# Pixie8888/R3DFSSeg

Hardware: NVIDIA B200
Metric: MPTI episodes/s (2-way 5-shot, 2048 pts) (higher is better)
Workload: dtype f32

## Files before the change

r3dfsseg_b200/csrc/lp.cu:

```cuda
#include <cooperative_groups.h>

#include <stdlib.h>

#include "common.cuh"
#include "lp.cuh"

namespace cg = cooperative_groups;

#define GD_BM 128
#define GD_BN 64
#define GD_BK 16

template <int ROWS, int KC>
__device__ __forceinline__ void lp_load_tile_T(float* __restrict__ dst,
                                               const float* __restrict__ src, int ld, int64_t row0,
                                               int64_t rows_end, int k0, int k_end) {
  constexpr int KG = KC / 8;
  constexpr int PAIRS = (ROWS / 4) * KG;
  const int lane = threadIdx.x & 31, w = threadIdx.x >> 5;
  const int nw = blockDim.x >> 5;
  const int r_lo = lane & 3, k_lo = lane >> 2;
  for (int p = w; p < PAIRS; p += nw) {
    int kg = p % KG, rg = p / KG;
    int row = 4 * rg + r_lo, kk = 8 * kg + k_lo;
// ... 911 lines not shown
  float v[NCV];
#pragma unroll
  for (int c = 0; c < NCV; ++c) v[c] = warp_sum(part[c]);
  if (lane == 0) {
#pragma unroll
    for (int c = 0; c < NCV; ++c) s_warp[w * CG_MAXC + c] = v[c];
  }
  __syncthreads();
  const int par = xcnt & 1;
  if (tid < NCV) {
    float s = 0.f;
    for (int q = 0; q < n_warps; ++q) s += s_warp[q * CG_MAXC + tid];
    for (int r = 0; r < CL; ++r) {
      float* dst = cluster.map_shared_rank(&ex->slot[par][rank][tid], r);
      *dst = s;
    }
  }
  cluster.sync();
#pragma unroll
  for (int c = 0; c < NCV; ++c) {
    float s = 0.f;
    for (int r = 0; r < CL; ++r) s += ex->slot[par][r][c];
    total[c] = s;
  }
  ++xcnt;
}

__global__ __launch_bounds__(256) void cg_hist_kernel(const int32_t* __restrict__ rowptr,
                                                      const int32_t* __restrict__ rowlen,
                                                      const uint8_t* __restrict__ valid,
                                                      const uint16_t* __restrict__ mcol, int nn,
                                                      int k, int32_t* __restrict__ rowmax) {
  const int g = blockIdx.y;
  const int i = blockIdx.x * 8 + (threadIdx.x >> 5);
  if (i >= nn) return;
  const int lane = threadIdx.x & 31;
  const int64_t vb = (int64_t)g * nn;
  int mx = 0;
  if (valid[vb + i]) {
    const int L = rowlen[vb + i];
    const uint16_t* c = mcol + vb * lp_rowcap(k) + rowptr[vb + i];
    int cnt[8] = {0, 0, 0, 0, 0, 0, 0, 0};
    for (int t0 = 0; t0 < L; t0 += 32) {
      const int t = t0 + lane;
      const int res = t < L ? (int)(c[t] & 7) : -1;
#pragma unroll
      for (int b = 0; b < 8; ++b) cnt[b] += __popc(__ballot_sync(0xffffffffu, res == b));
    }
#pragma unroll
    for (int b = 0; b < 8; ++b) mx = max(mx, cnt[b]);
  }
  if (lane == 0) rowmax[vb + i] = mx;
}

__global__ __launch_bounds__(1024) void cg_pack_kernel(
    const int32_t* __restrict__ rowptr, const int32_t* __restrict__ rowlen,
    const int32_t* __restrict__ rowmax, const uint16_t* __restrict__ mcol,
    const float* __restrict__ mval, int nn, int k, int64_t pk_cap, int32_t* __restrict__ tab_all,
    int32_t* __restrict__ flags, uint2* __restrict__ pcol, float4* __restrict__ pval) {
  extern __shared__ __align__(16) unsigned char pk_smem[];
  uint32_t* s_key = reinterpret_cast<uint32_t*>(pk_smem);
  int* s_pre = reinterpret_cast<int*>(s_key + 4096);
  int* s_prx = s_pre + 8192;
  __shared__ int s_scan[2][32];
  __shared__ int s_tot[2];
  __shared__ int s_rng[2];
  __shared__ int s_wtot[32], s_wbase[32];
  const int CL = gridDim.x, rank = blockIdx.x, g = blockIdx.y;
  const int tid = threadIdx.x, lane = tid & 31, w = tid >> 5;
  const int64_t vb = (int64_t)g * nn;
  const int32_t* rp = rowptr + vb;
  const int32_t* rl = rowlen + vb;
  const int32_t* rmx = rowmax + vb;
  const uint16_t* mc = mcol + vb * lp_rowcap(k);
  const float* mv = mval + vb * lp_rowcap(k);
  int32_t* tab = tab_all + (size_t)(g * CL + rank) * CG_TAB_INTS;
  for (int e = tid; e < CG_TAB_HDR + 32 * CG_MAXPASS * 2; e += 1024) tab[e] = 0;
  {
    int nseg[8], run = 0, runx = 0;
#pragma unroll
    for (int u = 0; u < 8; ++u) {
      const int i = tid * 8 + u;
      nseg[u] = i < nn ? (rmx[i] + CG_SEGR - 1) / CG_SEGR : 0;
      run += nseg[u];
      runx += nseg[u] > 1 ? nseg[u] : 0;
    }
    int inc = run, incx = runx;
#pragma unroll
    for (int o = 1; o < 32; o <<= 1) {
      const int a = __shfl_up_sync(0xffffffffu, inc, o), ax = __shfl_up_sync(0xffffffffu, incx, o);
      if (lane >= o) {
        inc += a;
        incx += ax;
      }
    }
    if (lane == 31) {
      s_scan[0][w] = inc;
      s_scan[1][w] = incx;
    }
    __syncthreads();
    if (w == 0) {
      int v = s_scan[0][lane], vx = s_scan[1][lane];
      int i2 = v, ix2 = vx;
#pragma unroll
      for (int o = 1; o < 32; o <<= 1) {
        const int a = __shfl_up_sync(0xffffffffu, i2, o), ax = __shfl_up_sync(0xffffffffu, ix2, o);
        if (lane >= o) {
          i2 += a;
          ix2 += ax;
        }
      }
      s_scan[0][lane] = i2 - v;
      s_scan[1][lane] = ix2 - vx;
      if (lane == 31) {
        s_tot[0] = i2;
        s_tot[1] = ix2;
      }
    }
    if (tid == 0) {
      s_rng[0] = nn;
      s_rng[1] = 0;
    }
    __syncthreads();
    int pre = s_scan[0][w] + inc - run, prex = s_scan[1][w] + incx - runx;
#pragma unroll
    for (int u = 0; u < 8; ++u) {
      const int i = tid * 8 + u;
      if (i < nn) {
        s_pre[i] = pre;
        s_prx[i] = prex;
      }
      pre += nseg[u];
      prex += nseg[u] > 1 ? nseg[u] : 0;
    }
  }
  __syncthreads();
  const int NV = s_tot[0];
  for (int i = tid; i < nn; i += 1024) {
    const int owner = NV > 0 ? min(CL - 1, (int)((int64_t)s_pre[i] * CL / NV)) : (i * CL) / nn;
    if (owner == rank) {
      atomicMin(&s_rng[0], i);
      atomicMax(&s_rng[1], i + 1);
    }
  }
  __syncthreads();
  const int lo = min(s_rng[0], s_rng[1]), hi = s_rng[1];
  const int pre_lo = lo < nn ? s_pre[lo] : NV, prx_lo = lo < nn ? s_prx[lo] : s_tot[1];
  const int nv = (hi < nn ? s_pre[hi] : NV) - pre_lo;
  const int nx = (hi < nn ? s_prx[hi] : s_tot[1]) - prx_lo;
  const int passes = (nv + CGC_MAXT - 1) / CGC_MAXT;
  const int64_t share = pk_cap / CL;
  bool bad = passes > CG_MAXPASS || nx > CG_MAXPART || hi - lo > 8191;
  int npow = 32;
  while (npow < nv) npow <<= 1;
  if (!bad) {
    for (int i = tid; i < npow; i += 1024) s_key[i] = 0;
    __syncthreads();
    for (int i = lo + tid; i < hi; i += 1024) {
      const int mx = rmx[i];
      const int ns = (mx + CG_SEGR - 1) / CG_SEGR;
      if (ns > 255) bad = true;
      for (int sg = 0; sg < ns && sg < 256; ++sg) {
        const int ranks = min(CG_SEGR, mx - sg * CG_SEGR);
        s_key[s_pre[i] - pre_lo + sg] =
            ((uint32_t)(2 * ranks) << 21) | ((uint32_t)(i - lo) << 8) | (uint32_t)sg;
      }
    }
  }
  bad = __syncthreads_or(bad);
  if (!bad) {
    for (int ksz = 2; ksz <= npow; ksz <<= 1)
      for (int j = ksz >> 1; j > 0; j >>= 1) {
        for (int i = tid; i < npow; i += 1024) {
          const int ixj = i ^ j;
          if (ixj > i) {
            const uint32_t x = s_key[i], y = s_key[ixj];
            const bool desc = (i & ksz) == 0;
            if (desc ? x < y : x > y) {
              s_key[i] = y;
              s_key[ixj] = x;
            }
          }
        }
        __syncthreads();
      }
    if (tid < 32) {
      int tot = 0;
      for (int p = 0; p < passes; ++p) {
        const int i0 = p * CGC_MAXT + tid * 32;
        tot += i0 < nv ? (int)(s_key[i0] >> 21) * 32 : 0;
      }
      s_wtot[tid] = tot;
    }
    __syncthreads();
    if (tid == 0) {
      int run = 0;
      for (int q = 0; q < 32; ++q) {
        s_wbase[q] = run;
        run += s_wtot[q];
      }
      s_tot[0] = run;
    }
    __syncthreads();
    if (s_tot[0] > share) bad = true;
  }
  if (tid == 0) {
    tab[0] = lo;
    tab[1] = hi;
    tab[2] = bad ? 0 : passes;
    tab[3] = nx;
    if (bad) atomicOr(&flags[g], 1);
  }
  if (bad) return;
  for (int e = tid; e < CG_MAXPASS * CGC_MAXT; e += 1024) {
    const int p = e / CGC_MAXT, t = e % CGC_MAXT;
    const int i = p * CGC_MAXT + t;
    int m0 = -1, m1 = 0;
    if (p < passes && i < nv) {
      const uint32_t key = s_key[i];
      const int rloc = (int)((key >> 8) & 0x1fffu), sg = (int)(key & 0xffu);
      const int ns = (rmx[lo + rloc] + CG_SEGR - 1) / CG_SEGR;
      m0 = (rloc << 8) | sg;
      m1 = (ns << 16) | (ns > 1 ? s_prx[lo + rloc] - prx_lo : 0);
    }
    tab[CG_TAB_HDR + 32 * CG_MAXPASS * 2 + 2 * e + 0] = m0;
    tab[CG_TAB_HDR + 32 * CG_MAXPASS * 2 + 2 * e + 1] = m1;
  }
  uint2* gc = pcol + (int64_t)g * pk_cap + rank * share;
  float4* gv = pval + (int64_t)g * pk_cap + rank * share;
  int base = s_wbase[w];
  for (int p = 0; p < passes; ++p) {
    const int i0 = p * CGC_MAXT + w * 32;
    const int rounds = i0 < nv ? (int)(s_key[i0] >> 21) : 0;
    if (lane == 0) {
      tab[CG_TAB_HDR + (w * CG_MAXPASS + p) * 2 + 0] = (int)(rank * share) + base;
      tab[CG_TAB_HDR + (w * CG_MAXPASS + p) * 2 + 1] = rounds;
    }
    for (int r = 0; r < rounds; ++r) {
      const unsigned t0 = (unsigned)(lane + 4 * r);
      uint2 c2;
      c2.x = (t0 & 7u) | (((t0 + 1) & 7u) << 16);
      c2.y = ((t0 + 2) & 7u) | (((t0 + 3) & 7u) << 16);
      gc[base + r * 32 + lane] = c2;
      gv[base + r * 32 + lane] = make_float4(0.f, 0.f, 0.f, 0.f);
    }
    __syncwarp();
    uint16_t* c16 = reinterpret_cast<uint16_t*>(gc + base);
    float* v32 = reinterpret_cast<float*>(gv + base);
    int my_L = 0, my_ptr = 0, my_sg = 0;
    if (i0 + lane < nv) {
      const uint32_t key = s_key[i0 + lane];
      const int row = lo + (int)((key >> 8) & 0x1fffu);
      my_L = rl[row];
      my_ptr = rp[row];
      my_sg = (int)(key & 0xffu);
    }
    const int n_here = min(32, nv - i0);
    for (int l = 0; l < n_here; ++l) {
      const int L = __shfl_sync(0xffffffffu, my_L, l), sg = __shfl_sync(0xffffffffu, my_sg, l);
      const int ptr = __shfl_sync(0xffffffffu, my_ptr, l);
      const int r_lo = sg * CG_SEGR, r_hi = r_lo + CG_SEGR;
      const uint16_t* c = mc + ptr;
      const float* v = mv + ptr;
      int seen[8] = {0, 0, 0, 0, 0, 0, 0, 0};
      int col_n = lane < L ? (int)c[lane] : -1;
      float val_n = lane < L ? v[lane] : 0.f;
      for (int t0 = 0; t0 < L; t0 += 32) {
        const int col = col_n;
        const float val = val_n;
        const int tn = t0 + 32 + lane;
        col_n = tn < L ? (int)c[tn] : -1;
        val_n = tn < L ? v[tn] : 0.f;
        const int res = col >= 0 ? (col & 7) : -1;
        int rho = -1;
#pragma unroll
        for (int b = 0; b < 8; ++b) {
          const uint32_t m = __ballot_sync(0xffffffffu, res == b);
          if (res == b) rho = seen[b] + __popc(m & ((1u << lane) - 1));
          seen[b] += __popc(m);
        }
        if (rho >= r_lo && rho < r_hi) {
          const int step = 8 * (rho - r_lo) + ((res - l) & 7);
          const int64_t d = ((int64_t)(step >> 2) * 32 + l) * 4 + (step & 3);
          c16[d] = (uint16_t)col;
          v32[d] = val;
        }
        int done_all = 1;
#pragma unroll
        for (int b = 0; b < 8; ++b) done_all &= seen[b] >= r_hi;
        if (done_all) break;
      }
    }
    __syncwarp();
    base += rounds * 32;
  }
}

template <int NCV>
__global__ __launch_bounds__(CGC_MAXT, 1) void lp_cg_kernel(
    const int32_t* __restrict__ rowptr, const int32_t* __restrict__ rowlen,
    const uint16_t* __restrict__ mcol, const float* __restrict__ mval,
    const uint8_t* __restrict__ valid, int nn, int k,
    const float* __restrict__ Y, int nc, float alpha, float tol, int max_iter,
    float* __restrict__ Z, float* __restrict__ X, float* __restrict__ R, float* __restrict__ Pv,
    float* __restrict__ AP, int32_t* __restrict__ iters_out, float* __restrict__ resid_out,
    const int32_t* __restrict__ tab_all, const int32_t* __restrict__ flags,
    const uint2* __restrict__ pcol, const float4* __restrict__ pval, int64_t pk_cap) {
  cg::cluster_group cluster = cg::this_cluster();
  const int CL = cluster.num_blocks(), rank = cluster.block_rank();
  const int g = blockIdx.y;
  extern __shared__ __align__(16) float Ps[];
  __shared__ CgExchange ex;
  __shared__ float s_warp[(CGC_MAXT / 32) * CG_MAXC];
  float* s_split = Ps + (size_t)nn * NCV;
  const int tid = threadIdx.x, lane = tid & 31, w = tid >> 5, T = blockDim.x;
  const int64_t vb = (int64_t)g * nn;
  const uint8_t* vg = valid + vb;
  const float* Yg = Y + vb * nc;
  float* Zg = Z + vb * nc;
  float* Xg = X + vb * NCV;
  float* Rg = R + vb * NCV;
  float* Pg = Pv + vb * NCV;
  float* APg = AP + vb * NCV;
  const int32_t* tab = tab_all + (size_t)(g * CL + rank) * CG_TAB_INTS;
  const int lo = tab[0], hi = tab[1];
  const int nloc = hi - lo;
  int xcnt = 0;

  float part[NCV], bb[NCV], rs[NCV], tot[NCV];
#pragma unroll
  for (int c = 0; c < NCV; ++c) part[c] = 0.f;
  for (int jj = tid; jj < nloc; jj += T) {
    const int row = lo + jj;
    const bool ok = vg[row];
#pragma unroll
    for (int c = 0; c < NCV; ++c) {
      const float y = (ok && c < nc) ? Yg[(int64_t)row * nc + c] : 0.f;
      Xg[(int64_t)row * NCV + c] = 0.f;
      Rg[(int64_t)row * NCV + c] = y;
      Pg[(int64_t)row * NCV + c] = y;
      APg[(int64_t)row * NCV + c] = 0.f;
      part[c] = fmaf(y, y, part[c]);
    }
  }
  cg_allreduce<NCV>(cluster, &ex, s_warp, part, xcnt, bb);
  bool done[NCV];
  bool all_done = true;
#pragma unroll
  for (int c = 0; c < NCV; ++c) {
    rs[c] = bb[c];
    done[c] = !(bb[c] > 0.f);
    all_done = all_done && done[c];
  }
  const float tol2 = tol * tol;
  const bool packed = flags[g] == 0;
  const int passes = packed ? tab[2] : 0;
  const bool any_split = packed && tab[3] > 0;
  const int32_t* t_slice = tab + CG_TAB_HDR + w * CG_MAXPASS * 2;
  const int32_t* t_thread = tab + CG_TAB_HDR + 32 * CG_MAXPASS * 2 + 2 * tid;
  const uint2* gc = pcol + (int64_t)g * pk_cap;
  const float4* gv = pval + (int64_t)g * pk_cap;
  int it = 0;
  while (!all_done && it < max_iter) {
    {
      const float4* src = reinterpret_cast<const float4*>(Pg);
      float4* dst = reinterpret_cast<float4*>(Ps);
      const int n4 = nn * (NCV / 4);
      for (int i = tid; i < n4; i += T) dst[i] = __ldcg(src + i);
    }
    __syncthreads();
#pragma unroll
    for (int c = 0; c < NCV; ++c) part[c] = 0.f;
    if (packed) {
      constexpr unsigned SH = NCV == 4 ? 4 : 5;
      const unsigned char* Pb = reinterpret_cast<const unsigned char*>(Ps);
#pragma unroll
      for (int p = 0; p < passes; ++p) {
        const int rounds = __ldg(t_slice + 2 * p + 1);
        if (rounds == 0) continue;
        const int sbase = __ldg(t_slice + 2 * p);
        const uint2* c2 = gc + sbase + lane;
        const float4* v4 = gv + sbase + lane;
        float acc[NCV];
#pragma unroll
        for (int c = 0; c < NCV; ++c) acc[c] = 0.f;
        auto fma4 = [&](float wgt, unsigned byte_off) {
#pragma unroll
          for (int q = 0; q < NCV / 4; ++q) {
            const float4 p4 = *reinterpret_cast<const float4*>(Pb + byte_off + 16 * q);
            acc[4 * q + 0] = fmaf(wgt, p4.x, acc[4 * q + 0]);
            acc[4 * q + 1] = fmaf(wgt, p4.y, acc[4 * q + 1]);
            acc[4 * q + 2] = fmaf(wgt, p4.z, acc[4 * q + 2]);
            acc[4 * q + 3] = fmaf(wgt, p4.w, acc[4 * q + 3]);
          }
        };
        auto consume = [&](const uint2& c, const float4& v) {
          fma4(v.x, (c.x & 0xffffu) << SH);
          fma4(v.y, (c.x >> 16) << SH);
          fma4(v.z, (c.y & 0xffffu) << SH);
          fma4(v.w, (c.y >> 16) << SH);
        };
        uint2 ca = __ldcs(c2), cb = __ldcs(c2 + 32);
        float4 va = __ldcs(v4), vb4 = __ldcs(v4 + 32);
        for (int r = 2; r < rounds; r += 2) {
          const uint2 na = __ldcs(c2 + r * 32), nb = __ldcs(c2 + r * 32 + 32);
          const float4 wa = __ldcs(v4 + r * 32), wb = __ldcs(v4 + r * 32 + 32);
          consume(ca, va);
          consume(cb, vb4);
          ca = na;
          cb = nb;
          va = wa;
          vb4 = wb;
        }
        consume(ca, va);
        consume(cb, vb4);
        const int m0 = __ldg(t_thread + 2 * p * CGC_MAXT), m1 = __ldg(t_thread + 2 * p * CGC_MAXT + 1);
        if (m0 >= 0) {
          if ((m1 >> 16) == 1) {
            const int row = lo + (m0 >> 8);
#pragma unroll
            for (int c = 0; c < NCV; ++c) {
              const float pv = Ps[(size_t)row * NCV + c];
              const float ap = pv - alpha * acc[c];
              APg[(int64_t)row * NCV + c] = ap;
              part[c] = fmaf(pv, ap, part[c]);
            }
          } else {
            float* dst = s_split + (size_t)((m1 & 0xffff) + (m0 & 0xff)) * NCV;
#pragma unroll
            for (int c = 0; c < NCV; ++c) dst[c] = acc[c];
          }
        }
      }
      if (any_split) {
        __syncthreads();
        for (int p = 0; p < passes; ++p) {
          const int m0 = __ldg(t_thread + 2 * p * CGC_MAXT), m1 = __ldg(t_thread + 2 * p * CGC_MAXT + 1);
          if (m0 >= 0 && (m1 >> 16) > 1 && (m0 & 0xff) == 0) {
            const int row = lo + (m0 >> 8), ns = m1 >> 16;
            const float* src = s_split + (size_t)(m1 & 0xffff) * NCV;
#pragma unroll
            for (int c = 0; c < NCV; ++c) {
              float sum = 0.f;
              for (int sg = 0; sg < ns; ++sg) sum += src[sg * NCV + c];
              const float pv = Ps[(size_t)row * NCV + c];
              const float ap = pv - alpha * sum;
              APg[(int64_t)row * NCV + c] = ap;
              part[c] = fmaf(pv, ap, part[c]);
            }
          }
        }
      }
    } else {
      const int32_t* rp = rowptr + vb;
      const int32_t* rl = rowlen + vb;
      const uint16_t* mc = mcol + vb * lp_rowcap(k);
      const float* mv = mval + vb * lp_rowcap(k);
      for (int row = lo + w; row < hi; row += T >> 5) {
        if (!vg[row]) continue;
        float acc[NCV];
#pragma unroll
        for (int c = 0; c < NCV; ++c) acc[c] = 0.f;
        const int L = rl[row];
        const uint16_t* crow = mc + rp[row];
        const float* vrow = mv + rp[row];
        for (int t = lane; t < L; t += 32) {
          const int cj = (int)crow[t];
          const float cv = vrow[t];
#pragma unroll
          for (int c = 0; c < NCV; ++c) acc[c] = fmaf(cv, Ps[(size_t)cj * NCV + c], acc[c]);
        }
#pragma unroll
        for (int c = 0; c < NCV; ++c) {
          const float sum = warp_sum(acc[c]);
          const float pv = Ps[(size_t)row * NCV + c];
          const float ap = pv - alpha * sum;
          if (lane == 0) {
            APg[(int64_t)row * NCV + c] = ap;
            part[c] = fmaf(pv, ap, part[c]);
          }
        }
      }
    }
    cg_allreduce<NCV>(cluster, &ex, s_warp, part, xcnt, tot);
    float a[NCV];
#pragma unroll
    for (int c = 0; c < NCV; ++c) a[c] = (!done[c] && tot[c] > 0.f) ? rs[c] / tot[c] : 0.f;
#pragma unroll
    for (int c = 0; c < NCV; ++c) part[c] = 0.f;
    for (int jj = tid; jj < nloc; jj += T) {
      const int row = lo + jj;
#pragma unroll
      for (int c = 0; c < NCV; ++c) {
        const int64_t o = (int64_t)row * NCV + c;
        const float r = Rg[o] - a[c] * APg[o];
        Xg[o] = fmaf(a[c], Ps[o], Xg[o]);
        Rg[o] = r;
        part[c] = fmaf(r, r, part[c]);
      }
    }
    cg_allreduce<NCV>(cluster, &ex, s_warp, part, xcnt, tot);
    float beta[NCV];
    all_done = true;
#pragma unroll
    for (int c = 0; c < NCV; ++c) {
      beta[c] = (!done[c] && rs[c] > 0.f) ? tot[c] / rs[c] : 0.f;
      if (!done[c]) {
        rs[c] = tot[c];
        if (tot[c] <= tol2 * bb[c]) done[c] = true;
      }
      all_done = all_done && done[c];
    }
    for (int jj = tid; jj < nloc; jj += T) {
      const int row = lo + jj;
#pragma unroll
      for (int c = 0; c < NCV; ++c)
        if (!done[c]) {
          const int64_t o = (int64_t)row * NCV + c;
          Pg[o] = fmaf(beta[c], Ps[o], Rg[o]);
        }
    }
    ++it;
    cluster.sync();
  }
  for (int jj = tid; jj < nloc; jj += T) {
    const int row = lo + jj;
    for (int c = 0; c < nc; ++c) Zg[(int64_t)row * nc + c] = Xg[(int64_t)row * NCV + c];
  }
  if (rank == 0 && tid == 0) {
    if (iters_out) iters_out[g] = it;
    if (resid_out) {
      float m = 0.f;
#pragma unroll
      for (int c = 0; c < NCV; ++c)
        if (bb[c] > 0.f) m = fmaxf(m, sqrtf(rs[c] / bb[c]));
      resid_out[g] = m;
    }
  }
  cluster.sync();
}

template <int NCV>
static int launch_cg(int CL, int G, size_t smem, cudaStream_t st, const int32_t* rowptr,
                     const int32_t* rowlen, const uint16_t* mcol, const float* mval,
                     const uint8_t* valid, int nn, int k, const float* Y, int nc,
                     float alpha, float tol, int max_iter, float* Z, float* X, float* R, float* P,
                     float* AP, int32_t* iters_out, float* resid_out, void* scratch,
                     size_t scratch_bytes) {
  cudaError_t e = cudaFuncSetAttribute(lp_cg_kernel<NCV>,
                                       cudaFuncAttributeMaxDynamicSharedMemorySize, 200 * 1024);
  if (e != cudaSuccess) return (int)e;
  if (CL > 8) {
    e = cudaFuncSetAttribute(lp_cg_kernel<NCV>, cudaFuncAttributeNonPortableClusterSizeAllowed, 1);
    if (e != cudaSuccess) return (int)e;
  }
  const int T = CGC_MAXT;
  smem += sizeof(float) * (size_t)CG_MAXPART * NCV;
  cudaLaunchConfig_t cfg = {};
  cfg.gridDim = dim3(CL, G, 1);
  cfg.blockDim = dim3(T, 1, 1);
  cfg.dynamicSmemBytes = smem;
  cfg.stream = st;
  cudaLaunchAttribute attr[1];
  attr[0].id = cudaLaunchAttributeClusterDimension;
  attr[0].val.clusterDim.x = CL;
  attr[0].val.clusterDim.y = 1;
  attr[0].val.clusterDim.z = 1;
  cfg.attrs = attr;
  cfg.numAttrs = 1;
  {
    int n_clusters = 0;
    e = cudaOccupancyMaxActiveClusters(&n_clusters, lp_cg_kernel<NCV>, &cfg);
    if (e != cudaSuccess || n_clusters < 1) {
      (void)cudaGetLastError();
      return -1000;
    }
  }
  const int64_t pk_cap = lp_pack_groups(nn, k);
  const size_t tab_bytes = align_up(sizeof(int32_t) * (size_t)G * CL * CG_TAB_INTS, 256);
  const size_t flg_bytes = align_up(sizeof(int32_t) * (size_t)G * (1 + nn), 256);
  const size_t col_bytes = align_up(sizeof(uint2) * (size_t)G * pk_cap, 256);
  const size_t val_bytes = align_up(sizeof(float4) * (size_t)G * pk_cap, 256);
  if (!scratch || scratch_bytes < tab_bytes + flg_bytes + col_bytes + val_bytes)
    return R3DFS_E_WORKSPACE;
  unsigned char* sp = reinterpret_cast<unsigned char*>(scratch);
  int32_t* tab = reinterpret_cast<int32_t*>(sp);
  int32_t* flags = reinterpret_cast<int32_t*>(sp + tab_bytes);
  uint2* pcol = reinterpret_cast<uint2*>(sp + tab_bytes + flg_bytes);
  float4* pval = reinterpret_cast<float4*>(sp + tab_bytes + flg_bytes + col_bytes);
  e = cudaMemsetAsync(flags, 0, sizeof(int32_t) * (size_t)G, st);
  if (e != cudaSuccess) return (int)e;
  e = cudaFuncSetAttribute(cg_pack_kernel, cudaFuncAttributeMaxDynamicSharedMemorySize, CG_PK_SMEM);
  if (e != cudaSuccess) return (int)e;
  int32_t* rowmax = flags + G;
  cg_hist_kernel<<<dim3((nn + 7) / 8, G), 256, 0, st>>>(rowptr, rowlen, valid, mcol, nn, k, rowmax);
  R3DFS_CHECK_LAUNCH();
  cg_pack_kernel<<<dim3(CL, G), 1024, CG_PK_SMEM, st>>>(rowptr, rowlen, rowmax, mcol, mval, nn, k,
                                                       pk_cap, tab, flags, pcol, pval);
  R3DFS_CHECK_LAUNCH();
  const int32_t* tabc = tab;
  const int32_t* flc = flags;
  const uint2* pc = pcol;
  const float4* pv = pval;
  e = cudaLaunchKernelEx(&cfg, lp_cg_kernel<NCV>, rowptr, rowlen, mcol, mval, valid, nn, k, Y, nc,
                         alpha, tol, max_iter, Z, X, R, P, AP, iters_out, resid_out, tabc, flc, pc,
                         pv, pk_cap);
  if (e != cudaSuccess) return (int)e;
  ++r3dfs_launches;
  return 0;
}

#define GCG_SLOT 8
#define GCG_MAX_GS 160

__device__ __forceinline__ unsigned ld_acquire_u32(const unsigned* p) {
  unsigned v;
  asm volatile("ld.acquire.gpu.global.u32 %0, [%1];" : "=r"(v) : "l"(p) : "memory");
  return v;
}

__device__ __forceinline__ void group_barrier(unsigned* cnt, unsigned& target, int GS) {
  __syncthreads();
  if (threadIdx.x == 0) {
    target += (unsigned)GS;
    __threadfence();
    atomicAdd(cnt, 1u);
    while (ld_acquire_u32(cnt) < target) {
    }
    __threadfence();
  }
  __syncthreads();
}

template <int NCV>
__device__ __forceinline__ void group_allreduce(float* s_warp, float* s_slot, const float* part,
                                                float* slots, int rank, int GS, unsigned* cnt,
                                                unsigned& target, int& phase, float* total) {
  const int tid = threadIdx.x, lane = tid & 31, w = tid >> 5;
  float v[NCV];
#pragma unroll
  for (int c = 0; c < NCV; ++c) v[c] = warp_sum(part[c]);
  if (lane == 0) {
#pragma unroll
    for (int c = 0; c < NCV; ++c) s_warp[w * CG_MAXC + c] = v[c];
  }
  __syncthreads();
  float* my = slots + ((size_t)(phase & 1) * GS + rank) * GCG_SLOT;
  if (tid < NCV) {
    float s = 0.f;
    for (int q = 0; q < CG_THREADS / 32; ++q) s += s_warp[q * CG_MAXC + tid];
    __stcg(my + tid, s);
  }
  group_barrier(cnt, target, GS);
  const float* all = slots + (size_t)(phase & 1) * GS * GCG_SLOT;
  if (tid < GS) {
#pragma unroll
    for (int q = 0; q < NCV / 4; ++q)
      reinterpret_cast<float4*>(s_slot + tid * GCG_SLOT)[q] =
          __ldcg(reinterpret_cast<const float4*>(all + (size_t)tid * GCG_SLOT) + q);
  }
  __syncthreads();
#pragma unroll
  for (int c = 0; c < NCV; ++c) total[c] = 0.f;
  for (int r = 0; r < GS; ++r) {
#pragma unroll
    for (int q = 0; q < NCV / 4; ++q) {
      const float4 t4 = reinterpret_cast<const float4*>(s_slot + r * GCG_SLOT)[q];
      total[4 * q + 0] += t4.x;
      total[4 * q + 1] += t4.y;
      total[4 * q + 2] += t4.z;
      total[4 * q + 3] += t4.w;
    }
  }
  ++phase;
}

template <int NCV, bool SMEM>
__device__ __forceinline__ void cg_row_product(const uint16_t* crow, const float* vrow, int L,
                                               int lane, const float* Ps, float* acc) {
  int t0 = 0;
  for (; t0 + 256 <= L; t0 += 256) {
    int cj[8];
    float cv[8];
#pragma unroll
    for (int u = 0; u < 8; ++u) {
      const int t = t0 + lane + 32 * u;
      cj[u] = (int)crow[t];
      cv[u] = vrow[t];
    }
#pragma unroll
    for (int u = 0; u < 8; ++u) {
#pragma unroll
      for (int q = 0; q < NCV / 4; ++q) {
        const float4 p4 = *reinterpret_cast<const float4*>(Ps + (int64_t)cj[u] * NCV + 4 * q);
        acc[4 * q + 0] = fmaf(cv[u], p4.x, acc[4 * q + 0]);
        acc[4 * q + 1] = fmaf(cv[u], p4.y, acc[4 * q + 1]);
        acc[4 * q + 2] = fmaf(cv[u], p4.z, acc[4 * q + 2]);
        acc[4 * q + 3] = fmaf(cv[u], p4.w, acc[4 * q + 3]);
      }
    }
  }
  if (t0 < L) {
    const int nU = (L - t0 + 31) >> 5;
    int cj[8];
    float cv[8];
#pragma unroll
    for (int u = 0; u < 8; ++u) {
      const int t = t0 + lane + 32 * u;
      const bool ok = u < nU && t < L;
      cj[u] = ok ? (int)crow[t] : 0;
      cv[u] = ok ? vrow[t] : 0.f;
    }
#pragma unroll
    for (int u = 0; u < 8; ++u) {
      if (u < nU) {
#pragma unroll
        for (int q = 0; q < NCV / 4; ++q) {
          const float4 p4 = *reinterpret_cast<const float4*>(Ps + (int64_t)cj[u] * NCV + 4 * q);
          acc[4 * q + 0] = fmaf(cv[u], p4.x, acc[4 * q + 0]);
          acc[4 * q + 1] = fmaf(cv[u], p4.y, acc[4 * q + 1]);
          acc[4 * q + 2] = fmaf(cv[u], p4.z, acc[4 * q + 2]);
          acc[4 * q + 3] = fmaf(cv[u], p4.w, acc[4 * q + 3]);
        }
      }
    }
  }
}

template <int NCV>
__global__ __launch_bounds__(CG_THREADS, 1) void lp_cg_group_kernel(
    const int32_t* __restrict__ rowptr, const int32_t* __restrict__ rowlen,
    const uint16_t* __restrict__ mcol, const float* __restrict__ mval,
    const uint8_t* __restrict__ valid, int G, int nn, int k, const float* __restrict__ Y, int nc,
    float alpha, float tol, int max_iter, float* __restrict__ Z, float* __restrict__ Pv,
    unsigned* __restrict__ counters, float* __restrict__ slots_all, int GS, int rows_max,
    int cache_entries, int32_t* __restrict__ iters_out, float* __restrict__ resid_out) {
  extern __shared__ __align__(16) unsigned char smem_raw[];
  float* Ps = reinterpret_cast<float*>(smem_raw);
  float* xs = Ps + (size_t)nn * NCV;
  float* rsm = xs + (size_t)rows_max * NCV;
  float* aps = rsm + (size_t)rows_max * NCV;
  int* s_off = reinterpret_cast<int*>(aps + (size_t)rows_max * NCV);
  float* c_val = reinterpret_cast<float*>(s_off + rows_max);
  uint16_t* c_col = reinterpret_cast<uint16_t*>(c_val + cache_entries);
  __shared__ float s_warp[(CG_THREADS / 32) * CG_MAXC];
  __shared__ __align__(16) float s_slot[GCG_MAX_GS * GCG_SLOT];
  const int tid = threadIdx.x, lane = tid & 31, w = tid >> 5;
  const int group = blockIdx.x / GS, rank = blockIdx.x % GS, n_groups = gridDim.x / GS;
  if (group >= n_groups) return;
  unsigned* cnt = counters + group * 32;
  float* slots = slots_all + (size_t)group * 2 * GS * GCG_SLOT;
  unsigned target = 0;
  int phase = 0;
  const int chunk = (nn + GS - 1) / GS;
  const int lo = min(nn, rank * chunk), hi = min(nn, lo + chunk);
  const int nrows = hi - lo;
  const float tol2 = tol * tol;

  for (int g = group; g < G; g += n_groups) {
    const int64_t vb = (int64_t)g * nn;
    const uint8_t* vg = valid + vb;
    const float* Yg = Y + vb * nc;
    float* Zg = Z + vb * nc;
    float* Pg = Pv + vb * NCV;
    const int32_t* rp = rowptr + vb;
    const int32_t* rl = rowlen + vb;
    const uint16_t* mc = mcol + vb * lp_rowcap(k);
    const float* mv = mval + vb * lp_rowcap(k);
    if (w == 0) {
      int base = 0;
      for (int r0 = 0; r0 < nrows; r0 += 32) {
        const int r = r0 + lane;
        const int L = (r < nrows && vg[lo + r]) ? rl[lo + r] : 0;
        int incl = L;
#pragma unroll
        for (int o = 1; o < 32; o <<= 1) {
          const int a = __shfl_up_sync(0xffffffffu, incl, o);
          if (lane >= o) incl += a;
        }
        const int off = base + incl - L;
        if (r < nrows) s_off[r] = (off + L <= cache_entries) ? off : -1;
        base += __shfl_sync(0xffffffffu, incl, 31);
      }
    }
    __syncthreads();
    for (int r = w; r < nrows; r += CG_THREADS / 32) {
      const int off = s_off[r];
      if (off < 0 || !vg[lo + r]) continue;
      const int L = rl[lo + r];
      const uint16_t* crow = mc + rp[lo + r];
      const float* vrow = mv + rp[lo + r];
      for (int t = lane; t < L; t += 32) {
        c_col[off + t] = crow[t];
        c_val[off + t] = vrow[t];
      }
    }
    float part[NCV], bb[NCV], rs[NCV], tot[NCV];
#pragma unroll
    for (int c = 0; c < NCV; ++c) part[c] = 0.f;
    for (int r = tid; r < nrows; r += CG_THREADS) {
      const int row = lo + r;
      const bool ok = vg[row];
      float y[NCV];
#pragma unroll
      for (int c = 0; c < NCV; ++c) {
        y[c] = (ok && c < nc) ? Yg[(int64_t)row * nc + c] : 0.f;
        xs[r * NCV + c] = 0.f;
        rsm[r * NCV + c] = y[c];
        aps[r * NCV + c] = 0.f;
        part[c] = fmaf(y[c], y[c], part[c]);
      }
#pragma unroll
      for (int q = 0; q < NCV / 4; ++q)
        __stcg(reinterpret_cast<float4*>(Pg + (int64_t)row * NCV) + q,
               make_float4(y[4 * q], y[4 * q + 1], y[4 * q + 2], y[4 * q + 3]));
    }
    group_allreduce<NCV>(s_warp, s_slot, part, slots, rank, GS, cnt, target, phase, bb);
    bool done[NCV];
    bool all_done = true;
#pragma unroll
    for (int c = 0; c < NCV; ++c) {
      rs[c] = bb[c];
      done[c] = !(bb[c] > 0.f);
      all_done = all_done && done[c];
    }
    int it = 0;
    while (!all_done && it < max_iter) {
      {
        const float4* src = reinterpret_cast<const float4*>(Pg);
        float4* dst = reinterpret_cast<float4*>(Ps);
        const int n4 = nn * (NCV / 4);
        for (int i4 = tid; i4 < n4; i4 += CG_THREADS) dst[i4] = __ldcg(src + i4);
      }
      __syncthreads();
#pragma unroll
      for (int c = 0; c < NCV; ++c) part[c] = 0.f;
      for (int r = w; r < nrows; r += CG_THREADS / 32) {
        const int row = lo + r;
        if (!vg[row]) continue;
        float acc[NCV];
#pragma unroll
        for (int c = 0; c < NCV; ++c) acc[c] = 0.f;
        const int L = rl[row];
        const int off = s_off[r];
        if (off >= 0)
          cg_row_product<NCV, true>(c_col + off, c_val + off, L, lane, Ps, acc);
        else
          cg_row_product<NCV, false>(mc + rp[row], mv + rp[row], L, lane, Ps, acc);
#pragma unroll
        for (int c = 0; c < NCV; ++c) {
          const float s = warp_sum(acc[c]);
          const float p = Ps[(int64_t)row * NCV + c];
          const float ap = p - alpha * s;
          if (lane == 0) {
            aps[r * NCV + c] = ap;
            part[c] = fmaf(p, ap, part[c]);
          }
        }
      }
      group_allreduce<NCV>(s_warp, s_slot, part, slots, rank, GS, cnt, target, phase, tot);
      float a[NCV];
#pragma unroll
      for (int c = 0; c < NCV; ++c) a[c] = (!done[c] && tot[c] > 0.f) ? rs[c] / tot[c] : 0.f;
#pragma unroll
      for (int c = 0; c < NCV; ++c) part[c] = 0.f;
      for (int r = tid; r < nrows; r += CG_THREADS) {
#pragma unroll
        for (int c = 0; c < NCV; ++c) {
          const int o = r * NCV + c;
          const float rr = rsm[o] - a[c] * aps[o];
          xs[o] = fmaf(a[c], Ps[(int64_t)(lo + r) * NCV + c], xs[o]);
          rsm[o] = rr;
          part[c] = fmaf(rr, rr, part[c]);
        }
      }
      group_allreduce<NCV>(s_warp, s_slot, part, slots, rank, GS, cnt, target, phase, tot);
      float beta[NCV];
      all_done = true;
#pragma unroll
      for (int c = 0; c < NCV; ++c) {
        beta[c] = (!done[c] && rs[c] > 0.f) ? tot[c] / rs[c] : 0.f;
        if (!done[c]) {
          rs[c] = tot[c];
          if (tot[c] <= tol2 * bb[c]) done[c] = true;
        }
        all_done = all_done && done[c];
      }
      ++it;
      if (all_done || it >= max_iter) break;
      for (int r = tid; r < nrows; r += CG_THREADS) {
        const int row = lo + r;
        float pn[NCV];
#pragma unroll
        for (int c = 0; c < NCV; ++c) {
          const float pold = Ps[(int64_t)row * NCV + c];
          pn[c] = done[c] ? pold : fmaf(beta[c], pold, rsm[r * NCV + c]);
        }
#pragma unroll
        for (int q = 0; q < NCV / 4; ++q)
          __stcg(reinterpret_cast<float4*>(Pg + (int64_t)row * NCV) + q,
                 make_float4(pn[4 * q], pn[4 * q + 1], pn[4 * q + 2], pn[4 * q + 3]));
      }
      group_barrier(cnt, target, GS);
    }
    for (int r = tid; r < nrows; r += CG_THREADS)
      for (int c = 0; c < nc; ++c) Zg[(int64_t)(lo + r) * nc + c] = xs[r * NCV + c];
    if (rank == 0 && tid == 0) {
      if (iters_out) iters_out[g] = it;
      if (resid_out) {
        float m = 0.f;
#pragma unroll
        for (int c = 0; c < NCV; ++c)
          if (bb[c] > 0.f) m = fmaxf(m, sqrtf(rs[c] / bb[c]));
        resid_out[g] = m;
      }
    }
    __syncthreads();
  }
}

template <int NCV>
static int launch_cg_group(int G, cudaStream_t st, const int32_t* rowptr, const int32_t* rowlen,
                           const uint16_t* mcol, const float* mval, const uint8_t* valid, int nn,
                           int k, const float* Y, int nc, float alpha, float tol, int max_iter,
                           float* Z, float* P, float* scratch, size_t scratch_floats,
                           int32_t* iters_out, float* resid_out) {
  static int n_sm = 0, coop = 0, smem_max = 0;
  if (n_sm == 0) {
    int dev = 0;
    cudaGetDevice(&dev);
    cudaDeviceGetAttribute(&coop, cudaDevAttrCooperativeLaunch, dev);
    cudaDeviceGetAttribute(&smem_max, cudaDevAttrMaxSharedMemoryPerBlockOptin, dev);
    cudaDeviceGetAttribute(&n_sm, cudaDevAttrMultiProcessorCount, dev);
  }
  if (!coop || n_sm < 8) return -1000;
  static const int gs_env = [] {
    const char* e = R3DFS_GETENV("R3DFS_CG_GROUP");
    return e ? atoi(e) : 0;
  }();
  int n_groups = gs_env > 0 ? min(32, max(1, n_sm / gs_env)) : min(G, 4);
  int GS = min(GCG_MAX_GS, gs_env > 0 ? gs_env : min(74, n_sm / n_groups));
  const int rows_max = (nn + GS - 1) / GS;
  const size_t fixed = sizeof(float) * ((size_t)nn * NCV + 3 * (size_t)rows_max * NCV) +
                       sizeof(int) * (size_t)rows_max;
  const size_t smem = (size_t)smem_max - 8 * 1024;
  if (fixed + 6 * 1024 > smem) return -1000;
  const int cache_entries = (int)(((smem - fixed) / 6) & ~(size_t)7);
  const size_t need_scratch = 32 * 32 + (size_t)n_groups * 2 * GS * GCG_SLOT;
  if (need_scratch > scratch_floats) return -1000;
  cudaError_t e = cudaFuncSetAttribute(lp_cg_group_kernel<NCV>,
                                       cudaFuncAttributeMaxDynamicSharedMemorySize, (int)smem);
  if (e != cudaSuccess) return (int)e;
  e = cudaMemsetAsync(scratch, 0, 32 * 32 * sizeof(unsigned), st);
  if (e != cudaSuccess) return (int)e;
  unsigned* counters = reinterpret_cast<unsigned*>(scratch);
  float* slots = scratch + 32 * 32;
  int grid = n_groups * GS;
  void* args[] = {(void*)&rowptr, (void*)&rowlen, (void*)&mcol, (void*)&mval, (void*)&valid,
                  (void*)&G, (void*)&nn, (void*)&k, (void*)&Y, (void*)&nc, (void*)&alpha,
                  (void*)&tol, (void*)&max_iter, (void*)&Z, (void*)&P, (void*)&counters,
                  (void*)&slots, (void*)&GS, (void*)&rows_max, (void*)&cache_entries,
                  (void*)&iters_out, (void*)&resid_out};
  e = cudaLaunchCooperativeKernel((const void*)lp_cg_group_kernel<NCV>, dim3(grid), dim3(CG_THREADS),
                                  args, smem, st);
  if (e != cudaSuccess) {
    (void)cudaGetLastError();
    return -1000;
  }
  ++r3dfs_launches;
  return 0;
}

__global__ __launch_bounds__(1024) void query_head_kernel(const float* __restrict__ Z, int nn,
                                                          int q_off, int nq, int nc,
                                                          const int64_t* __restrict__ qy,
                                                          float* __restrict__ logits,
                                                          float* __restrict__ loss,
                                                          int32_t* __restrict__ pred) {
  __shared__ float s_red[32];
  const int g = blockIdx.x, tid = threadIdx.x;
  const float* Zg = Z + ((int64_t)g * nn + q_off) * nc;
  float part = 0.f;
  for (int i = tid; i < nq; i += 1024) {
    float mx = -INFINITY;
    int am = 0;
    for (int c = 0; c < nc; ++c) {
      const float v = Zg[(int64_t)i * nc + c];
      logits[((int64_t)g * nq + i) * nc + c] = v;
      if (v > mx) {
        mx = v;
        am = c;
      }
    }
    if (pred) pred[(int64_t)g * nq + i] = am;
    if (qy) {
      float se = 0.f;
      for (int c = 0; c < nc; ++c) se += expf(Zg[(int64_t)i * nc + c] - mx);
      const int y = (int)qy[(int64_t)g * nq + i];
      part += (mx + logf(se)) - Zg[(int64_t)i * nc + y];
    }
  }
  part = warp_sum(part);
  if ((tid & 31) == 0) s_red[tid >> 5] = part;
  __syncthreads();
  if (tid == 0 && loss) {
    float s = 0.f;
    for (int q = 0; q < 32; ++q) s += s_red[q];
    loss[g] = qy ? s / (float)nq : 0.f;
  }
}

__global__ void confusion_kernel(const int32_t* __restrict__ pred, const int64_t* __restrict__ gt,
                                 const int32_t* __restrict__ class_slot, int n_way,
                                 int64_t pts_per_episode, int64_t total, int n_slots,
                                 unsigned long long* __restrict__ counters) {
  const int64_t e = (int64_t)blockIdx.x * blockDim.x + threadIdx.x;
  if (e >= total) return;
  const int64_t ep = e / pts_per_episode;
  const int g = (int)gt[e], p = pred[e];
  const int gi = g == 0 ? 0 : class_slot[ep * n_way + g - 1];
  const int pi = p == 0 ? 0 : class_slot[ep * n_way + p - 1];
  atomicAdd(&counters[gi], 1ull);
  atomicAdd(&counters[n_slots + pi], 1ull);
  if (g == p) atomicAdd(&counters[2 * n_slots + gi], 1ull);
}

int launch_affinity(const float* F, int64_t graph_rows, int64_t row_off, const uint8_t* valid,
                    int G, int nn, int D, int k, float sigma, float* norms, float* D2, int32_t* nbr,
                    float* sim, cudaStream_t st, const StageRec* sr) {
  if (D % 4 != 0 || D > 32 * LP_MAX_F4 || k > 1024 || nn > 65535) return R3DFS_E_UNSUPPORTED;
  R3DFS_TRY(launch_row_norms_batched(F + row_off * D, graph_rows * D, G, nn, D, D, norms, st));
  if (simt_gemm_forced()) {
    dim3 gd((nn + GD_BM - 1) / GD_BM, (nn + GD_BN - 1) / GD_BN, G);
    gram_dist_kernel<<<gd, 256, 0, st>>>(F, graph_rows, row_off, nn, D, norms, D2);
    R3DFS_CHECK_LAUNCH();
  } else {
    static const bool dist_tc = R3DFS_GETENV("R3DFS_DIST_TC") != nullptr;
    int rc = dist_tc ? R3DFS_E_UNSUPPORTED
                     : launch_gram_dist_ts(F, graph_rows, row_off, G, nn, D, norms, D2, st);
    if (rc == R3DFS_E_UNSUPPORTED)
      rc = launch_gram_dist_tc(F, graph_rows, row_off, G, nn, D, norms, D2, st);
    R3DFS_TRY(rc);
  }
  if (sr) sr->mark(R3DFS_ST_DIST, st);
  static const bool sel_block = R3DFS_GETENV("R3DFS_SELECT_BLOCK") != nullptr;
  if (nn <= 32 * 80 && !sel_block) {
    const dim3 gs((nn + SELW_WARPS - 1) / SELW_WARPS, G);
    if (nn <= 32 * 40)
      knn_select_warp_kernel<40><<<gs, SELW_WARPS * 32, 0, st>>>(D2, valid, nn, k, nbr);
    else
      knn_select_warp_kernel<80><<<gs, SELW_WARPS * 32, 0, st>>>(D2, valid, nn, k, nbr);
    R3DFS_CHECK_LAUNCH();
  } else if (nn <= 31 * SEL_THREADS && !sel_block) {
    const size_t smem = sizeof(unsigned) * (size_t)nn;
    static const bool sel_256 = R3DFS_GETENV("R3DFS_SELECT_256") != nullptr;
    static const bool sel_512 = R3DFS_GETENV("R3DFS_SELECT_512") != nullptr;
    if (nn <= 19 * SEL_THREADS && !sel_512)
      knn_select_reg_kernel<20><<<dim3(nn, G), SEL_THREADS, smem, st>>>(D2, valid, nn, k, nbr);
    else if (!sel_256)
      knn_select_reg_kernel<20, 512><<<dim3(nn, G), 512, smem, st>>>(D2, valid, nn, k, nbr);
    else
      knn_select_reg_kernel<32><<<dim3(nn, G), SEL_THREADS, smem, st>>>(D2, valid, nn, k, nbr);
    R3DFS_CHECK_LAUNCH();
  } else {
    size_t smem = sizeof(unsigned) * (size_t)nn;
    cudaError_t e = cudaFuncSetAttribute(knn_select_kernel,
                                         cudaFuncAttributeMaxDynamicSharedMemorySize, (int)smem);
    if (e != cudaSuccess) return (int)e;
    knn_select_kernel<<<dim3(nn, G), SEL_THREADS, smem, st>>>(D2, valid, nn, k, nbr);
    R3DFS_CHECK_LAUNCH();
  }
  if (sr) sr->mark(R3DFS_ST_SELECT, st);
  edge_sim_kernel<<<dim3((nn + 7) / 8, G), 256, 0, st>>>(F, graph_rows, row_off, nn, D, valid, nbr,
                                                        k, sigma, sim);
  R3DFS_CHECK_LAUNCH();
  if (sr) sr->mark(R3DFS_ST_SIM, st);
  return 0;
}

int launch_lp_solve(const int32_t* rowptr, const int32_t* rowlen, const uint16_t* mcol,
                    const float* mval, const uint8_t* valid, int G, int nn, int k, const float* Y,
                    int nc, float alpha, float tol, int max_iter, float* Z, float* X, float* R,
                    float* P, float* AP, int32_t* iters_out, float* resid_out, cudaStream_t st,
                    bool latency, void* scratch, size_t scratch_bytes) {
  if (nc > CG_MAXC || nc < 1 || nn > 8192) return R3DFS_E_UNSUPPORTED;
  const int ncv = nc <= 4 ? 4 : 8;
  const size_t smem_cg = sizeof(float) * (size_t)nn * ncv;
  if (smem_cg > 200 * 1024) return R3DFS_E_UNSUPPORTED;
  int rc = -1000;
  static const bool no_group = R3DFS_GETENV("R3DFS_CG_NOGROUP") != nullptr;
  if (latency && !no_group) {
    const size_t scratch_floats = (size_t)G * nn * ncv;
    rc = ncv == 4 ? launch_cg_group<4>(G, st, rowptr, rowlen, mcol, mval, valid, nn, k, Y, nc, alpha,
                                       tol, max_iter, Z, P, AP, scratch_floats, iters_out, resid_out)
                  : launch_cg_group<8>(G, st, rowptr, rowlen, mcol, mval, valid, nn, k, Y, nc, alpha,
                                       tol, max_iter, Z, P, AP, scratch_floats, iters_out, resid_out);
    if (rc == 0) return 0;
    if (rc != -1000) return rc;
  }
  static const int cl_first = [] {
    const char* e = R3DFS_GETENV("R3DFS_CG_CLUSTER");
    const int v = e ? atoi(e) : 0;
    return (v == 16 || v == 8 || v == 4 || v == 2) ? v : 0;
  }();
  int dev = 0, n_sm = 0;
  cudaGetDevice(&dev);
  cudaDeviceGetAttribute(&n_sm, cudaDevAttrMultiProcessorCount, dev);
  const int rows_cta_max = CGC_MAXT * CG_MAXPASS;
  const int cl_need = (nn + rows_cta_max - 1) / rows_cta_max;
  int cl_start = cl_first ? cl_first : (G <= 4 ? 16 : max(1, min(8, n_sm / G)));
  cl_start = max(cl_start, cl_need);
  for (int CL = cl_start; CL >= cl_need && CL >= 1 && rc == -1000;
       CL = (CL & (CL - 1)) ? (1 << (31 - __builtin_clz(CL))) : CL >> 1) {
    if (ncv == 4)
      rc = launch_cg<4>(CL, G, smem_cg, st, rowptr, rowlen, mcol, mval, valid, nn, k, Y, nc, alpha,
                        tol, max_iter, Z, X, R, P, AP, iters_out, resid_out, scratch, scratch_bytes);
    else
      rc = launch_cg<8>(CL, G, smem_cg, st, rowptr, rowlen, mcol, mval, valid, nn, k, Y, nc, alpha,
                        tol, max_iter, Z, X, R, P, AP, iters_out, resid_out, scratch, scratch_bytes);
  }
  if (rc != 0) return rc == -1000 ? R3DFS_E_UNSUPPORTED : rc;
  return 0;
}

int launch_label_propagate(const int32_t* nbr, float* sim, const uint8_t* valid, int G, int nn,
                           int k, const float* Y, int nc, float alpha, float tol, int max_iter,
                           int32_t* in_cnt, int32_t* in_ptr, int32_t* in_src, float* in_w,
                           float* dinv, int32_t* rowptr, int32_t* rowlen, int32_t* cursor,
                           uint16_t* mcol, float* mval, float* Z, float* X, float* R, float* P,
                           float* AP, int32_t* iters_out, float* resid_out, cudaStream_t st,
                           const StageRec* sr, void* scratch, size_t scratch_bytes, bool latency,
                           void* dense_scratch, int32_t* dense_info) {
  if (nc > CG_MAXC || nc < 1 || nn > 8192) return R3DFS_E_UNSUPPORTED;
  cudaError_t e;
  const int64_t edges = (int64_t)nn * k;
  dim3 ge((unsigned)((edges + 255) / 256), G);
  const int W = (nn + 31) / 32;
  const size_t bits_bytes = sizeof(uint32_t) * (size_t)G * nn * W;
  const size_t pre_bytes = sizeof(uint16_t) * (size_t)G * nn * W;
  static const bool force_sort = R3DFS_GETENV("R3DFS_INEDGE_SORT") != nullptr;
  if (scratch && scratch_bytes >= bits_bytes + pre_bytes && !force_sort) {
    uint32_t* bits = reinterpret_cast<uint32_t*>(scratch);
    uint16_t* pre = reinterpret_cast<uint16_t*>(reinterpret_cast<unsigned char*>(scratch) + bits_bytes);
    e = cudaMemsetAsync(bits, 0, bits_bytes, st);
    if (e != cudaSuccess) return (int)e;
    in_bits_kernel<<<ge, 256, 0, st>>>(nbr, valid, nn, k, W, bits);
    R3DFS_CHECK_LAUNCH();
    in_rank_kernel<<<dim3((nn + 7) / 8, G), 256, 0, st>>>(bits, nn, W, pre, in_cnt);
    R3DFS_CHECK_LAUNCH();
    in_scan_kernel<<<G, 1024, 0, st>>>(in_cnt, nn, in_ptr);
    R3DFS_CHECK_LAUNCH();
    in_fill_rank_kernel<<<ge, 256, 0, st>>>(nbr, sim, valid, nn, k, W, bits, pre, in_ptr, in_src,
                                            in_w);
    R3DFS_CHECK_LAUNCH();
  } else {
    e = cudaMemsetAsync(in_cnt, 0, sizeof(int32_t) * (size_t)G * nn, st);
    if (e != cudaSuccess) return (int)e;
    in_count_kernel<<<ge, 256, 0, st>>>(nbr, valid, nn, k, in_cnt);
    R3DFS_CHECK_LAUNCH();
    in_scan_kernel<<<G, 1024, 0, st>>>(in_cnt, nn, in_ptr);
    R3DFS_CHECK_LAUNCH();
    in_fill_kernel<<<ge, 256, 0, st>>>(nbr, sim, valid, nn, k, in_ptr, in_cnt, in_src, in_w);
    R3DFS_CHECK_LAUNCH();
    e = cudaFuncSetAttribute(in_sort_kernel, cudaFuncAttributeMaxDynamicSharedMemorySize, 8 * 8192);
    if (e != cudaSuccess) return (int)e;
    in_sort_warp_kernel<<<dim3((nn + 7) / 8, G), 256, 0, st>>>(in_ptr, nn, k, in_src, in_w);
    R3DFS_CHECK_LAUNCH();
    in_sort_kernel<<<dim3(nn, G), 256, 8 * 1024, st>>>(in_ptr, nn, k, in_src, in_w, 256, 1024);
    R3DFS_CHECK_LAUNCH();
    in_sort_kernel<<<dim3(nn, G), 256, 8 * 8192, st>>>(in_ptr, nn, k, in_src, in_w, 1024, 8192);
    R3DFS_CHECK_LAUNCH();
  }
  dim3 gr((nn + 7) / 8, G);
  e = cudaMemsetAsync(cursor, 0, sizeof(int32_t) * (size_t)G, st);
  if (e != cudaSuccess) return (int)e;
  const size_t smem_m = (size_t)8 * k * 8;
  e = cudaFuncSetAttribute(merge_rows_kernel, cudaFuncAttributeMaxDynamicSharedMemorySize,
                           (int)smem_m);
  if (e != cudaSuccess) return (int)e;
  merge_rows_kernel<<<gr, 256, smem_m, st>>>(nbr, sim, in_ptr, in_src, in_w, valid, nn, k, cursor,
                                            rowptr, rowlen, mcol, mval);
  R3DFS_CHECK_LAUNCH();
  degree_merged_kernel<<<gr, 256, 0, st>>>(rowptr, rowlen, mval, nn, k, dinv);
  R3DFS_CHECK_LAUNCH();
  normalize_merged_kernel<<<gr, 256, 0, st>>>(rowptr, rowlen, mcol, mval, dinv, nn, k);
  R3DFS_CHECK_LAUNCH();
  if (sr) sr->mark(R3DFS_ST_SYM, st);

  if (dense_scratch) {
    R3DFS_TRY(launch_lp_cholesky_solve(rowptr, rowlen, mcol, mval, valid, G, nn, k, Y, nc, alpha, Z,
                                       dense_scratch, dense_info, st));
    if (sr) sr->mark(R3DFS_ST_CG, st);
    return 0;
  }
  R3DFS_TRY(launch_lp_solve(rowptr, rowlen, mcol, mval, valid, G, nn, k, Y, nc, alpha, tol, max_iter,
                            Z, X, R, P, AP, iters_out, resid_out, st, latency, scratch,
                            scratch_bytes));
  if (sr) sr->mark(R3DFS_ST_CG, st);
  return 0;
}

int launch_query_head(const float* Z, int G, int nn, int q_off, int nq, int nc, const int64_t* qy,
                      float* logits, float* loss, int32_t* pred, cudaStream_t st) {
  query_head_kernel<<<G, 1024, 0, st>>>(Z, nn, q_off, nq, nc, qy, logits, loss, pred);
  R3DFS_CHECK_LAUNCH();
  return 0;
}

int launch_confusion(const int32_t* pred, const int64_t* gt, const int32_t* class_slot, int E,
                     int n_way, int64_t pts, int n_slots, int64_t* counters, cudaStream_t st) {
  const int64_t total = (int64_t)E * pts;
  confusion_kernel<<<(unsigned)((total + 255) / 256), 256, 0, st>>>(
      pred, gt, class_slot, n_way, pts, total, n_slots,
      reinterpret_cast<unsigned long long*>(counters));
  R3DFS_CHECK_LAUNCH();
  return 0;
}
```

Baseline: 942.5.

## Broadcast CG search direction to cluster shared memory via DSMEM instead of global

```diff
diff --git a/r3dfsseg_b200/csrc/lp.cu b/r3dfsseg_b200/csrc/lp.cu
--- a/r3dfsseg_b200/csrc/lp.cu
+++ b/r3dfsseg_b200/csrc/lp.cu
@@ -1237,8 +1237,8 @@
     const uint16_t* __restrict__ mcol, const float* __restrict__ mval,
     const uint8_t* __restrict__ valid, int nn, int k,
     const float* __restrict__ Y, int nc, float alpha, float tol, int max_iter,
-    float* __restrict__ Z, float* __restrict__ X, float* __restrict__ R, float* __restrict__ Pv,
-    float* __restrict__ AP, int32_t* __restrict__ iters_out, float* __restrict__ resid_out,
+    float* __restrict__ Z, float* __restrict__ X, float* __restrict__ R, float* __restrict__ AP,
+    int32_t* __restrict__ iters_out, float* __restrict__ resid_out,
     const int32_t* __restrict__ tab_all, const int32_t* __restrict__ flags,
     const uint2* __restrict__ pcol, const float4* __restrict__ pval, int64_t pk_cap) {
   cg::cluster_group cluster = cg::this_cluster();
@@ -1255,28 +1255,38 @@
   float* Zg = Z + vb * nc;
   float* Xg = X + vb * NCV;
   float* Rg = R + vb * NCV;
-  float* Pg = Pv + vb * NCV;
   float* APg = AP + vb * NCV;
   const int32_t* tab = tab_all + (size_t)(g * CL + rank) * CG_TAB_INTS;
   const int lo = tab[0], hi = tab[1];
   const int nloc = hi - lo;
   int xcnt = 0;
 
+  auto publish_p = [&](int row, const float* p) {
+#pragma unroll
+    for (int q = 0; q < NCV / 4; ++q) {
+      const float4 v = make_float4(p[4 * q], p[4 * q + 1], p[4 * q + 2], p[4 * q + 3]);
+      for (int r = 0; r < CL; ++r)
+        reinterpret_cast<float4*>(cluster.map_shared_rank(Ps, r))[(size_t)row * (NCV / 4) + q] = v;
+    }
+  };
+  cluster.sync();
+
   float part[NCV], bb[NCV], rs[NCV], tot[NCV];
 #pragma unroll
   for (int c = 0; c < NCV; ++c) part[c] = 0.f;
   for (int jj = tid; jj < nloc; jj += T) {
     const int row = lo + jj;
     const bool ok = vg[row];
+    float y[NCV];
 #pragma unroll
     for (int c = 0; c < NCV; ++c) {
-      const float y = (ok && c < nc) ? Yg[(int64_t)row * nc + c] : 0.f;
+      y[c] = (ok && c < nc) ? Yg[(int64_t)row * nc + c] : 0.f;
       Xg[(int64_t)row * NCV + c] = 0.f;
-      Rg[(int64_t)row * NCV + c] = y;
-      Pg[(int64_t)row * NCV + c] = y;
+      Rg[(int64_t)row * NCV + c] = y[c];
       APg[(int64_t)row * NCV + c] = 0.f;
-      part[c] = fmaf(y, y, part[c]);
-    }
+      part[c] = fmaf(y[c], y[c], part[c]);
+    }
+    publish_p(row, y);
   }
   cg_allreduce<NCV>(cluster, &ex, s_warp, part, xcnt, bb);
   bool done[NCV];
@@ -1297,13 +1307,6 @@
   const float4* gv = pval + (int64_t)g * pk_cap;
   int it = 0;
   while (!all_done && it < max_iter) {
-    {
-      const float4* src = reinterpret_cast<const float4*>(Pg);
-      float4* dst = reinterpret_cast<float4*>(Ps);
-      const int n4 = nn * (NCV / 4);
-      for (int i = tid; i < n4; i += T) dst[i] = __ldcg(src + i);
-    }
-    __syncthreads();
 #pragma unroll
     for (int c = 0; c < NCV; ++c) part[c] = 0.f;
     if (packed) {
@@ -1448,12 +1451,13 @@
     }
     for (int jj = tid; jj < nloc; jj += T) {
       const int row = lo + jj;
-#pragma unroll
-      for (int c = 0; c < NCV; ++c)
-        if (!done[c]) {
-          const int64_t o = (int64_t)row * NCV + c;
-          Pg[o] = fmaf(beta[c], Ps[o], Rg[o]);
-        }
+      float pn[NCV];
+#pragma unroll
+      for (int c = 0; c < NCV; ++c) {
+        const int64_t o = (int64_t)row * NCV + c;
+        pn[c] = done[c] ? Ps[o] : fmaf(beta[c], Ps[o], Rg[o]);
+      }
+      publish_p(row, pn);
     }
     ++it;
     cluster.sync();
@@ -1479,7 +1483,7 @@
 static int launch_cg(int CL, int G, size_t smem, cudaStream_t st, const int32_t* rowptr,
                      const int32_t* rowlen, const uint16_t* mcol, const float* mval,
                      const uint8_t* valid, int nn, int k, const float* Y, int nc,
-                     float alpha, float tol, int max_iter, float* Z, float* X, float* R, float* P,
+                     float alpha, float tol, int max_iter, float* Z, float* X, float* R,
                      float* AP, int32_t* iters_out, float* resid_out, void* scratch,
                      size_t scratch_bytes) {
   cudaError_t e = cudaFuncSetAttribute(lp_cg_kernel<NCV>,
@@ -1538,7 +1542,7 @@
   const uint2* pc = pcol;
   const float4* pv = pval;
   e = cudaLaunchKernelEx(&cfg, lp_cg_kernel<NCV>, rowptr, rowlen, mcol, mval, valid, nn, k, Y, nc,
-                         alpha, tol, max_iter, Z, X, R, P, AP, iters_out, resid_out, tabc, flc, pc,
+                         alpha, tol, max_iter, Z, X, R, AP, iters_out, resid_out, tabc, flc, pc,
                          pv, pk_cap);
   if (e != cudaSuccess) return (int)e;
   ++r3dfs_launches;
@@ -2049,10 +2053,10 @@
        CL = (CL & (CL - 1)) ? (1 << (31 - __builtin_clz(CL))) : CL >> 1) {
     if (ncv == 4)
       rc = launch_cg<4>(CL, G, smem_cg, st, rowptr, rowlen, mcol, mval, valid, nn, k, Y, nc, alpha,
-                        tol, max_iter, Z, X, R, P, AP, iters_out, resid_out, scratch, scratch_bytes);
+                        tol, max_iter, Z, X, R, AP, iters_out, resid_out, scratch, scratch_bytes);
     else
       rc = launch_cg<8>(CL, G, smem_cg, st, rowptr, rowlen, mcol, mval, valid, nn, k, Y, nc, alpha,
-                        tol, max_iter, Z, X, R, P, AP, iters_out, resid_out, scratch, scratch_bytes);
+                        tol, max_iter, Z, X, R, AP, iters_out, resid_out, scratch, scratch_bytes);
   }
   if (rc != 0) return rc == -1000 ? R3DFS_E_UNSUPPORTED : rc;
   return 0;
```

New measurement: 949.3 (median of 6 runs). No clear change (+0.7%).
